# jltsiren/bwt-merge

Measured on AMD Instinct MI355X. Metric: merged Gbases/sec (input1+input2), bit-exact native BWT; value = inputs and result resident in HBM, host_to_host_value = SURVEY 8(d)'s T (page-locked host to page-locked host), higher is better.
Workload: dtype u64

## Files before the change

### bwt-merge_amd/csrc/api/context.hip.h

```cpp
#pragma once


namespace
{

thread_local std::string g_error;

int fail(int code, const char* fmt, ...)
{
  char buf[512];
  va_list ap; va_start(ap, fmt); vsnprintf(buf, sizeof(buf), fmt, ap); va_end(ap);
  g_error = buf;
  return code;
}

inline u64 div_up(u64 a, u64 b) { return (a + b - 1) / b; }

}


struct bwtm_context
{
  int device = -1;
  hipStream_t stream = nullptr;
  hipStream_t copy_stream = nullptr;
  std::recursive_mutex mu;
  bool is_default = false;
  std::atomic<long long> live_handles{0};

  bool profiling = false;
  std::string profile_only;
  bool profile_open = false;
  struct Pending { const char* name; hipEvent_t start, stop; };
  std::vector<Pending> pending;
  std::map<std::string, std::pair<double, uint64_t>> totals;
  std::vector<const char*> order;

  std::multimap<u64, void*> free_blocks;
  u64 cached_bytes = 0, held_bytes = 0, peak_bytes = 0;
  struct VBlock { u64 bytes = 0; std::vector<hipMemGenericAllocationHandle_t> chunks; hipEvent_t released = nullptr; };
  bool vmm = false;
  std::vector<hipMemGenericAllocationHandle_t> free_chunks;
  std::map<void*, VBlock> vblocks;
  u64 device_total = 0;
  u64 va_fallbacks = 0;

  void* stream_stage[4] = {nullptr, nullptr, nullptr, nullptr};
  u64 stream_stage_cap[4] = {0, 0, 0, 0};
  u64* host_scratch = nullptr;
  u64 scan1_tiles = 0, pull_scan1_tiles = 0;
};

namespace
{

struct Tuning
{
  long long search_algo = 0;
  long long frontier_unfused = 0;
  long long l1_cap = 0;
  long long emit_path = 0;
  long long round_emits = 1ll << 33;
  long long emit_budget = 0;
  long long frontier_epoch = 512;
  long long eager_cum_budget = 16ll << 30;
  long long upload_chunk = 256ll << 20;
  long long download_chunk = 128ll << 20;
  long long range_ratio = 8;
#ifdef BWTM_EXPERIMENTAL
  long long search_view = 0;
#endif
  long long frontier_stage_out = 1;
  long long frontier_parts = 0;
  long long part_capacity = 0;
  long long recs_uniform = 0;
  long long recs_window = 0;
  long long stream_samples_query = 0;
  long long stream_upload = 0;
  long long extract_batch = 1ll << 20;
  long long ingest_verify = 0;
#ifdef BWTM_DIAGNOSTICS
  long long walk_emit = 0;
  long long walk_blocks = 0;
  long long walk_kernel = 0;
  long long walk_ablate = 0;
  long long walk_variant = 0;
  long long scatter_kernel = 0;
#endif
};
Tuning g_tune;

std::mutex g_registry_mu;
std::map<int, bwtm_context*> g_default_ctx;
thread_local bwtm_context* t_bound = nullptr;
thread_local bwtm_context* t_ctx = nullptr;

#define CTX (*t_ctx)

#define HIP_TRY(expr) do { hipError_t e_ = (expr); if(e_ != hipSuccess) { \
  return fail(e_ == hipErrorOutOfMemory ? BWTM_ENOMEM : BWTM_ENODEV, "%s failed: %s (%s:%d)", #expr, hipGetErrorString(e_), __FILE__, __LINE__); } } while(0)

#define TRY(expr) do { int rc_ = (expr); if(rc_ != BWTM_OK) { return rc_; } } while(0)

void vmm_setup(bwtm_context* c);
void pool_trim(bwtm_context* c);
void stream_stage_free(bwtm_context* c)
{
  for(int k = 0; k < 4; k++) { if(c->stream_stage[k]) { (void)hipHostFree(c->stream_stage[k]); } c->stream_stage[k] = nullptr; c->stream_stage_cap[k] = 0; }
}
void apply_env_tuning();

int context_setup(bwtm_context* c, int device)
{
  int count = 0;
  hipError_t e = hipGetDeviceCount(&count);
  if(e != hipSuccess || count <= 0) { return fail(BWTM_ENODEV, "no HIP device available (%s)", hipGetErrorString(e)); }
  if(device < 0 || device >= count) { return fail(BWTM_EINVAL, "device %d out of range (%d devices)", device, count); }
  HIP_TRY(hipSetDevice(device));
  apply_env_tuning();
  c->device = device;
  HIP_TRY(hipStreamCreateWithFlags(&c->stream, hipStreamNonBlocking));
  HIP_TRY(hipStreamCreateWithFlags(&c->copy_stream, hipStreamNonBlocking));
  HIP_TRY(hipHostMalloc((void**)&c->host_scratch, 128 * sizeof(u64), hipHostMallocDefault));
  vmm_setup(c);
  {
    hipDeviceProp_t prop;
    HIP_TRY(hipGetDeviceProperties(&prop, device));
    int per_cu_scan = 0, per_cu_pull = 0;
    HIP_TRY(hipOccupancyMaxActiveBlocksPerMultiprocessor(&per_cu_scan, (const void*)k_frontier_scan1, BLOCK_THREADS, 0));
    HIP_TRY(hipOccupancyMaxActiveBlocksPerMultiprocessor(&per_cu_pull, (const void*)k_pull_scan1, BLOCK_THREADS, 0));
    c->scan1_tiles = std::min<u64>(FRONTIER_SCAN1_TILES, (u64)std::max(per_cu_scan, 0) * (u64)std::max(prop.multiProcessorCount, 0));
    c->pull_scan1_tiles = std::min<u64>(FRONTIER_SCAN1_TILES, (u64)std::max(per_cu_pull, 0) * (u64)std::max(prop.multiProcessorCount, 0));
  }
  HIP_TRY(hipFuncSetAttribute((const void*)k_part_scatter_sorted, hipFuncAttributeMaxDynamicSharedMemorySize, 96 * 1024));
  HIP_TRY(hipFuncSetAttribute((const void*)k_lf_walk_binned<true>, hipFuncAttributeMaxDynamicSharedMemorySize, 40 * 1024));
#ifdef BWTM_DIAGNOSTICS
  HIP_TRY(hipFuncSetAttribute((const void*)k_lf_walk_lds<true>, hipFuncAttributeMaxDynamicSharedMemorySize, 122 * 1024));
  HIP_TRY(hipFuncSetAttribute((const void*)k_lf_walk_lds<false>, hipFuncAttributeMaxDynamicSharedMemorySize, 82 * 1024));
#endif
  return BWTM_OK;
}

void context_teardown(bwtm_context* c)
{
  if(c->device < 0) { return; }
  (void)hipSetDevice(c->device);
  if(c->stream) { (void)hipStreamSynchronize(c->stream); }
  if(c->copy_stream) { (void)hipStreamSynchronize(c->copy_stream); }
  for(auto& p : c->pending) { (void)hipEventDestroy(p.start); (void)hipEventDestroy(p.stop); }
  c->pending.clear();
  pool_trim(c);
  stream_stage_free(c);
  if(c->host_scratch) { (void)hipHostFree(c->host_scratch); }
  if(c->stream) { (void)hipStreamDestroy(c->stream); }
  if(c->copy_stream) { (void)hipStreamDestroy(c->copy_stream); }
}

int default_context(int device, bwtm_context** out)
{
  std::lock_guard<std::mutex> lock(g_registry_mu);
  auto it = g_default_ctx.find(device);
  if(it != g_default_ctx.end()) { *out = it->second; return BWTM_OK; }
  bwtm_context* c = new bwtm_context();
  c->is_default = true;
// ... 413 lines not shown

extern "C" void bwtm_context_destroy(bwtm_context* context)
{
  if(!context || context->is_default) { return; }
  if(t_bound == context) { t_bound = nullptr; }
  if(context->live_handles.load() > 0)
  {
    fail(BWTM_EINVAL, "bwtm_context_destroy: %lld handles of the context are still alive; context not destroyed", context->live_handles.load());
    return;
  }
  context_teardown(context);
  delete context;
}

extern "C" const char* bwtm_last_error(void) { return g_error.c_str(); }

namespace
{
int tune_set(const char* key, long long value)
{
  std::string k(key);
  if(k == "search_algo") { g_tune.search_algo = value; }
  else if(k == "frontier_unfused") { g_tune.frontier_unfused = value; }
  else if(k == "l1_cap") { g_tune.l1_cap = value; }
  else if(k == "emit_path") { g_tune.emit_path = value; }
  else if(k == "round_emits") { g_tune.round_emits = (value > 0 ? value : 1); }
  else if(k == "emit_budget") { g_tune.emit_budget = (value > 0 ? value : 0); }
  else if(k == "frontier_epoch") { g_tune.frontier_epoch = (value > 0 ? value : 512); }
  else if(k == "range_ratio") { g_tune.range_ratio = (value >= 0 ? value : 8); }
#ifdef BWTM_EXPERIMENTAL
  else if(k == "search_view") { g_tune.search_view = (value >= 0 && value <= 2 ? value : 0); }
#endif
  else if(k == "frontier_stage_out") { g_tune.frontier_stage_out = (value != 0); }
  else if(k == "frontier_parts") { g_tune.frontier_parts = (value > 0 ? value : 0); }
  else if(k == "stream_samples_query") { g_tune.stream_samples_query = (value != 0); }
  else if(k == "stream_upload") { g_tune.stream_upload = (value != 0); }
  else if(k == "ingest_verify") { g_tune.ingest_verify = (value != 0); }
  else if(k == "extract_batch") { g_tune.extract_batch = (value > 0 ? value : (1ll << 20)); }
  else if(k == "part_capacity") { g_tune.part_capacity = value; }
  else if(k == "recs_uniform") { g_tune.recs_uniform = (value > 0 ? 1 : (value < 0 ? -1 : 0)); }
  else if(k == "recs_window") { g_tune.recs_window = (value == 8192 || value == 16384 || value == 32768 ? value : 0); }
  else if(k == "eager_cum_budget") { g_tune.eager_cum_budget = (value > 0 ? value : (16ll << 30)); }
  else if(k == "upload_chunk") { g_tune.upload_chunk = (value > 0 ? value : (256ll << 20)); }
  else if(k == "download_chunk") { g_tune.download_chunk = (value > 0 ? value : (128ll << 20)); }
#ifdef BWTM_DIAGNOSTICS
  else if(k == "walk_emit") { g_tune.walk_emit = value; }
  else if(k == "walk_blocks") { g_tune.walk_blocks = value; }
  else if(k == "walk_kernel") { g_tune.walk_kernel = value; }
  else if(k == "walk_ablate") { g_tune.walk_ablate = value; }
  else if(k == "walk_variant") { g_tune.walk_variant = value; }
  else if(k == "scatter_kernel") { g_tune.scatter_kernel = value; }
#endif
  else { return fail(BWTM_EINVAL, "bwtm_tune: unknown key %s", key); }
  return BWTM_OK;
}

void apply_env_tuning()
{
  static std::mutex mu;
  static bool done = false;
  std::lock_guard<std::mutex> lock(mu);
  if(done) { return; }
  done = true;
  const char* env = std::getenv("BWTM_TUNE");
  if(!env) { return; }
  std::string all(env);
// ... 124 lines not shown
```

### bwt-merge_amd/csrc/api/search.hip.h

```cpp
#pragma once

struct bwtm_ra
{
  bwtm_context* ctx = nullptr;
  bwtm_ra() : ctx(t_ctx) { if(ctx) { ctx->live_handles++; } }
  ~bwtm_ra() { if(ctx) { ctx->live_handles--; } }
  bwtm_ra(const bwtm_ra&) = delete; bwtm_ra& operator=(const bwtm_ra&) = delete;
  u64 na = 0, nb = 0, n_out = 0;
  u64 nrecs_out = 0, nchunks = 0;
  DevBuf owned_bits;
  void* bits_ptr = nullptr;
  template<class T> T* bits_as() const { return (T*)bits_ptr; }
  DevBuf chunk_base;
  bool finalized = false;
  u64 values = 0;
  bool ranged = false;
  u64 range_first = 0, range_last = 0;
  DevBuf range_rel;
  DevBuf super_boff;
  bool windowed = false;
  u64 win_word_first = 0, win_words = 0;
};

#define WHOLE_RA(ra, who) if((ra)->windowed) { return fail(BWTM_EINVAL, who ": a window of a rank array (bwtm_ra_create_range) only serves the merge over partitioned records and the output-range entry points"); }
// ... 260 lines not shown
  {
    const u64 limit = std::max<u64>(1, std::min<u64>(count / (u64)g_tune.range_ratio, 1ull << 24));
    TRY(range_phase(a, b, seq_first, count, ra, limit, levels));
    if(levels.N == 0) { return BWTM_OK; }
    TRY(range_alive(levels, node_offsets));
    count = levels.alive;
    if(count == 0) { return BWTM_OK; }
  }
  const u64 ntiles = div_up(ra->n_out + 1, 1ull << TILE_SHIFT);
  const u64 nb_max = div_up(count, FR_BLOCK);
  const u64 nseg = 5 * nb_max;
  const u64 fcap = nb_max * FR_BLOCK;

  const u64 per_seq = b->n / (b->m > 0 ? b->m : 1) + 1;
  u64 emit_budget = (u64)g_tune.emit_budget;
  if(emit_budget == 0)
  {
    emit_budget = 16ull << 30;
    size_t free_b = 0, total_b = 0;
    if(hipMemGetInfo(&free_b, &total_b) == hipSuccess) { emit_budget = std::min<u64>(std::max<u64>(emit_budget, ((u64)free_b + CTX.cached_bytes) / 2), 64ull << 30); }
    else { (void)hipGetLastError(); }
  }
  u64 emit_cap = emit_budget / sizeof(unsigned short);
  if(emit_cap > b->n + 64) { emit_cap = b->n + 64; }
  if(emit_cap > 2 * count * per_seq + (1ull << 20)) { emit_cap = 2 * count * per_seq + (1ull << 20); }
  if(emit_cap < count) { emit_cap = count; }
  u64 EPOCH = std::max<u64>(1, (u64)g_tune.frontier_epoch);
  if(g_tune.l1_cap > 0) { emit_cap = (u64)g_tune.l1_cap; }
  else { EPOCH = std::max<u64>(1, std::min<u64>(EPOCH, emit_cap / std::max<u64>(count, 1))); }
  const u64 bound_budget = 2ull << 30;
  if(EPOCH * (ntiles + 1) * sizeof(u32) > bound_budget) { EPOCH = std::max<u64>(1, bound_budget / ((ntiles + 1) * sizeof(u32))); }

  const bool wide = (a->n >= (1ull << 32) || b->n >= (1ull << 32));
  DevBuf lo[2], hi[2], seg_len[2], seg_phys[2], seg_prefix, emit16, emit_base, bound;
  for(int k = 0; k < 2; k++)
  {
    TRY(lo[k].alloc(fcap * 8)); if(wide) { TRY(hi[k].alloc(fcap * 2)); }
    TRY(seg_len[k].alloc((nseg + 1) * sizeof(u64), true)); TRY(seg_phys[k].alloc((nseg + 1) * sizeof(u64), true));
  }
  TRY(seg_prefix.alloc((nseg + 1) * sizeof(u64)));
  DevBuf first_seg; TRY(first_seg.alloc((nb_max + 1) * sizeof(u32)));
  const u32 LOOK = (count >= (1ull << 24) ? 4 : (count >= (1ull << 20) ? 8 : 32));
  struct Events
  {
    hipEvent_t ev[32]; u32 n = 0;
    ~Events() { for(u32 k = 0; k < n; k++) { (void)hipEventDestroy(ev[k]); } }
  } events;
  for(u32 k = 0; k < LOOK; k++) { HIP_TRY(hipEventCreateWithFlags(&events.ev[k], hipEventDisableTiming)); events.n = k + 1; }
  const u64 scan_tiles = div_up(nseg + 1, (u64)SCAN_TILE);
  DevBuf scan_partial; TRY(scan_partial.alloc(scan_tiles * sizeof(u64), true));
  TRY(emit16.alloc((emit_cap + 16) * sizeof(unsigned short)));
  TRY(emit_base.alloc((EPOCH + 1) * sizeof(u64), true));
  TRY(bound.alloc(EPOCH * (ntiles + 1) * sizeof(u32)));
  HIP_TRY(hipMemsetAsync(bound.p, 0xFF, EPOCH * (ntiles + 1) * sizeof(u32), CTX.stream));

  if(node_phase)
  {
    TRY(range_expand(levels, node_offsets, lo[0].as<uint2>(), hi[0].as<unsigned short>()));
    LAUNCH("frontier_init", k_frontier_init_tables, div_up(nseg + 1, BLOCK_THREADS), BLOCK_THREADS, seg_len[0].as<u64>(), seg_phys[0].as<u64>(), nb_max, count);
    levels.release(); node_offsets.release();
  }
  else
  {
    u64 init_items = (fcap > nseg + 1 ? fcap : nseg + 1);
    LAUNCH("frontier_init", k_frontier_init, div_up(init_items, BLOCK_THREADS), BLOCK_THREADS, lo[0].as<uint2>(), hi[0].as<unsigned short>(),
      seg_len[0].as<u64>(), seg_phys[0].as<u64>(), nb_max, seq_first, count, a->m);
  }
  int cur = 0;
  u64 in_epoch = 0;
  u64 alive_bound = count, epoch_used = 0;
#ifdef BWTM_EXPERIMENTAL
  bool use_view = (g_tune.search_view == 1);
  if(g_tune.search_view == 2)
  {
    const u64 steps_left = (b->m > 0 ? b->n / b->m : 0);
    size_t free_b = 0, total_b = 0;
    const u64 need = (num_view_records(a->n) + num_view_records(b->n)) * 64;
    use_view = (count >= (1ull << 22) && steps_left >= 32 && hipMemGetInfo(&free_b, &total_b) == hipSuccess && (u64)free_b + CTX.cached_bytes > need + (8ull << 30));
    (void)hipGetLastError();
  }
  if(use_view)
  {
    int rc_view = ensure_view(a);
    if(rc_view == BWTM_OK) { rc_view = ensure_view(b); }
    if(rc_view != BWTM_OK) { use_view = false; }
  }
#endif
  u64 grid = nb_max;
  u64 written[2] = {nb_max, 0};
  u64* host_ring = nullptr;
  HIP_TRY(hipHostGetDevicePointer((void**)&host_ring, CTX.host_scratch + 64, 0));
  for(u64 t = 0; t <= b->n; t++)
  {
    bool size_in_ring = false;
    if(t >= LOOK)
    {
      HIP_TRY(hipEventSynchronize(events.ev[t % LOOK]));
      alive_bound = CTX.host_scratch[64 + (u32)(t % LOOK)];
      if(alive_bound == 0) { break; }
    }
    if(scan_tiles <= CTX.scan1_tiles && g_tune.frontier_unfused == 0)
    {
      LAUNCH("frontier_scan", k_frontier_scan1, scan_tiles, BLOCK_THREADS, seg_len[cur].as<const u64>(), scan_partial.as<unsigned long long>(), (u32)((t & 0x7FFFFFFFull) + 1), nseg,
        seg_prefix.as<u64>(), first_seg.as<u32>(), emit_base.as<u64>(), in_epoch, host_ring + (t % LOOK));
      size_in_ring = true;
    }
    else if(scan_tiles <= FRONTIER_SCAN_TILES && g_tune.frontier_unfused != 1)
    {
      if(scan_tiles > 1)
      {
        LAUNCH("scan_reduce", k_scan_reduce<0>, scan_tiles, BLOCK_THREADS, seg_len[cur].as<const u64>(), scan_partial.as<u64>(), nseg + 1, (u64)0, scan_tiles);
      }
      LAUNCH("frontier_scan", k_frontier_scan, scan_tiles, BLOCK_THREADS, seg_len[cur].as<const u64>(), scan_partial.as<const u64>(), nseg,
        seg_prefix.as<u64>(), first_seg.as<u32>(), emit_base.as<u64>(), in_epoch, host_ring + (t % LOOK));
      size_in_ring = true;
    }
    else
    {
      TRY(device_scan<0>(seg_len[cur].as<u64>(), seg_prefix.as<u64>(), nseg + 1));
      LAUNCH("frontier_prep", k_frontier_prep, div_up(nseg, BLOCK_THREADS), BLOCK_THREADS, seg_prefix.as<const u64>(), nseg, first_seg.as<u32>(),
        emit_base.as<u64>(), in_epoch);
    }
    if(!size_in_ring) { TRY(fetch_u64(seg_prefix.as<u64>() + nseg, 64 + (u32)(t % LOOK))); HIP_TRY(hipEventRecord(events.ev[t % LOOK], CTX.stream)); }
    {
      const u64 need = std::max<u64>(1, div_up(alive_bound, FR_BLOCK));
      if(g_tune.frontier_parts <= 1 && need * 4 < grid * 3) { grid = need; }
      const int nxt = 1 - cur;
      if(written[nxt] > grid)
      {
        for(u64 c = 0; c < 5; c++) { HIP_TRY(hipMemsetAsync(seg_len[nxt].as<u64>() + c * nb_max + grid, 0, (written[nxt] - grid) * sizeof(u64), CTX.stream)); }
      }
      written[nxt] = grid;
    }
    FrontierView f;
    f.lo = lo[cur].as<const uint2>(); f.hi = hi[cur].as<const unsigned short>();
    f.lo_next = lo[1 - cur].as<uint2>(); f.hi_next = hi[1 - cur].as<unsigned short>();
    f.seg_prefix = seg_prefix.as<const u64>(); f.seg_phys = seg_phys[cur].as<const u64>(); f.first_seg = first_seg.as<const u32>();
    f.seg_len_next = seg_len[1 - cur].as<u64>(); f.seg_phys_next = seg_phys[1 - cur].as<u64>();
    f.nb_max = nb_max;
    f.emit16 = emit16.as<unsigned short>(); f.emit_base = emit_base.as<const u64>(); f.emit_cap = emit_cap; f.bits32 = ra->bits_as<u32>();
    f.bound_row = bound.as<u32>() + in_epoch * (ntiles + 1); f.step = in_epoch; f.block_base = 0; f.src_lo = nullptr; f.src_hi = nullptr; f.nseg_in = 0;
#ifdef BWTM_DIAGNOSTICS
    if(g_tune.walk_emit == 1 && wide) { LAUNCH_STEP("frontier_step_noemit", 1, true, false, false, grid, a->view(), b->view(), f); }
    else if(g_tune.walk_emit == 1) { LAUNCH_STEP("frontier_step_noemit", 1, false, false, false, grid, a->view(), b->view(), f); }
    else
#endif
    if(g_tune.frontier_parts > 1)
    {
      const u64 parts = (u64)g_tune.frontier_parts, per = div_up(nb_max, parts);
      for(u64 part = 0; part < parts && part * per < nb_max; part++)
      {
        f.block_base = (u32)(part * per);
        const u64 nb_part = std::min<u64>(per, nb_max - part * per);
        const char* label = (part == 0 ? "frontier_step_slice0" : "frontier_step_slices");
        if(wide) { LAUNCH_STEP(label, 0, true, false, false, nb_part, a->view(), b->view(), f); }
        else { LAUNCH_STEP(label, 0, false, false, false, nb_part, a->view(), b->view(), f); }
      }
    }
#ifdef BWTM_EXPERIMENTAL
    else if(use_view && wide) { LAUNCH_STEP("frontier_step", 0, true, true, false, grid, a->view(), b->view(), f); }
    else if(use_view) { LAUNCH_STEP("frontier_step", 0, false, true, false, grid, a->view(), b->view(), f); }
#endif
    else if(wide) { LAUNCH_STEP("frontier_step", 0, true, false, false, grid, a->view(), b->view(), f); }
    else { LAUNCH_STEP("frontier_step", 0, false, false, false, grid, a->view(), b->view(), f); }
    if(size_in_ring) { HIP_TRY(hipEventRecord(events.ev[t % LOOK], CTX.stream)); }
    cur = 1 - cur;
    in_epoch++; epoch_used += alive_bound;
    if(in_epoch == EPOCH || (g_tune.l1_cap == 0 && epoch_used + alive_bound > emit_cap))
    {
      TRY(frontier_flush(ra, emit16, emit_cap, emit_base, bound, ntiles, in_epoch));
      HIP_TRY(hipMemsetAsync(bound.p, 0xFF, EPOCH * (ntiles + 1) * sizeof(u32), CTX.stream));
      HIP_TRY(hipMemsetAsync(emit_base.p, 0, (EPOCH + 1) * sizeof(u64), CTX.stream));
      in_epoch = 0; epoch_used = 0;
    }
  }
  TRY(frontier_flush(ra, emit16, emit_cap, emit_base, bound, ntiles, in_epoch));
  return BWTM_OK;
}

}


extern "C" uint64_t bwtm_ra_buffer_bytes(const bwtm_index* a, const bwtm_index* b)
{
  if(!a || !b) { return 0; }
  return div_up(num_records(a->n + b->n), 64) * CHUNK_WORDS * sizeof(u64);
}

extern "C" int bwtm_ra_create_on(const bwtm_index* a, const bwtm_index* b, void* device_buffer, uint64_t nbytes, bwtm_ra** out)
{
  if(!a || !b || !out) { return fail(BWTM_EINVAL, "bwtm_ra_create: null argument"); }
  if(a->ctx != b->ctx) { return fail(BWTM_EINVAL, "bwtm_ra_create: the two indexes live in different contexts"); }
  ENTER(a->ctx);
  bwtm_ra* ra = new bwtm_ra();
  ra->ctx = t_ctx;
// ... 170 lines not shown
```

### bwt-merge_amd/csrc/kernels/search_frontier.hip.h

```cpp
#pragma once


constexpr int FR_BLOCK = 256;
constexpr u32 PULL_SRC_SHIFT_ = 56;
constexpr u64 PULL_PHYS_MASK_ = (1ull << PULL_SRC_SHIFT_) - 1;
constexpr int FR_SEGS = 31;

struct FrontierView
{
  const uint2* lo; const unsigned short* hi;
  uint2* lo_next; unsigned short* hi_next;
  const u64* seg_prefix;
  const u64* seg_phys;
  const u32* first_seg;
  u64* seg_len_next; u64* seg_phys_next;
  u64 nb_max;
  unsigned short* emit16;
  const u64* emit_base;
  u64 emit_cap;
  u32* bits32;
  u32* bound_row;
  u64 step;
  u32 block_base;
  const uint2* const* src_lo; const unsigned short* const* src_hi;
  u64 nseg_in;
};

__global__ void __launch_bounds__(BLOCK_THREADS) k_frontier_init(uint2* lo, unsigned short* hi, u64* seg_len, u64* seg_phys, u64 nb_max,
  u64 seq_first, u64 count, u64 m_a)
{
  u64 g = (u64)blockIdx.x * BLOCK_THREADS + threadIdx.x;
  if(g < count)
  {
    u64 i = seq_first + g;
    lo[g] = make_uint2((u32)i, (u32)m_a);
    if(hi) { hi[g] = (unsigned short)(((i >> 32) & 0xFF) | (((m_a >> 32) & 0xFF) << 8)); }
  }
  if(g < 5 * nb_max)
  {
    u64 cls = g / nb_max, b = g % nb_max;
    u64 begin = b * FR_BLOCK;
    seg_len[g] = (cls == 0 && begin < count ? (count - begin < (u64)FR_BLOCK ? count - begin : (u64)FR_BLOCK) : 0);
    seg_phys[g] = begin;
  }
  if(g == 5 * nb_max) { seg_len[g] = 0; }
}

struct RecordFetch { uint4 v[4]; };

__device__ inline RecordFetch record_issue(const uint4* recs, u64 nrecs, u64 rec)
{
  RecordFetch rf;
  const uint4* p = recs + 4 * (rec < nrecs ? rec : nrecs - 1);
  rf.v[0] = p[0]; rf.v[1] = p[1]; rf.v[2] = p[2]; rf.v[3] = p[3];
  return rf;
}

__device__ inline void record_words(const RecordFetch& rf, u32 w[16])
{
#pragma unroll
  for(int k = 0; k < 4; k++) { w[4 * k] = rf.v[k].x; w[4 * k + 1] = rf.v[k].y; w[4 * k + 2] = rf.v[k].z; w[4 * k + 3] = rf.v[k].w; }
}

__device__ inline u64 ordinary_lf(const IndexView& X, u64 pos, u32& c, bool want_symbol)
{
  const uint4* p = X.recs + 4 * (pos >> REC_SHIFT);
  const u32 j = (u32)(pos & (REC_POS - 1));
  if(want_symbol)
  {
    const uint4 ch = p[j >> 5];
    const u32 t = j & 31;
    c = ((ch.x >> t) & 1u) | (((ch.y >> t) & 1u) << 1) | (((ch.z >> t) & 1u) << 2);
  }
  if(c == 0) { return 0; }
  u32 total = 0; u32 h[4];
#pragma unroll
  for(u32 k = 0; k < 4; k++)
  {
    const uint4 ch = p[k];
    total += (u32)__builtin_popcount(plane_match(ch.x, ch.y, ch.z, c) & below_mask(j, k));
    h[k] = ch.w;
  }
  const u32 sh = FIELD_BITS * (c - 1);
  const u64 lo = (u64)h[0] | ((u64)h[1] << 32), hi = (u64)h[2] | ((u64)h[3] << 32);
  u64 v;
  if(sh < 64) { v = lo >> sh; if(sh + FIELD_BITS > 64) { v |= hi << (64 - sh); } }
  else { v = hi >> (sh - 64); }
  return X.sup[(pos >> SUPER_SHIFT) * SUP_STRIDE + c] + ((u32)v & FIELD_MASK) + total;
}

template<int EMIT, bool HI, bool VIEW = false, bool PULL = false, bool STAGE = false>
__global__ void __launch_bounds__(FR_BLOCK, (VIEW ? 6 : 8)) k_frontier_step(IndexView A, IndexView B, FrontierView f)
{
  __shared__ u32 wave_cnt[FR_BLOCK / WAVE][6];
  __shared__ uint2 s_out[STAGE ? FR_BLOCK : 1];
  __shared__ unsigned short s_out_hi[STAGE && HI ? FR_BLOCK : 1];
  __shared__ u64 s_prefix[FR_SEGS + 1], s_phys[FR_SEGS + 1];
  __shared__ const uint2* s_src_lo[PULL ? 16 : 1];
  __shared__ const unsigned short* s_src_hi[PULL ? 16 : 1];
  const u64 nseg_out = 5 * f.nb_max;
  const u64 nseg = (PULL ? f.nseg_in : nseg_out);
  const u64 N = f.seg_prefix[nseg];
  const u32 bid = blockIdx.x + f.block_base;
  const u64 g0 = (u64)bid * FR_BLOCK;
  const u32 lane = lane_id(), wave = threadIdx.x >> 6;

  if(g0 >= N)
  {
    if(threadIdx.x < 5) { f.seg_len_next[(u64)threadIdx.x * f.nb_max + bid] = 0; f.seg_phys_next[(u64)threadIdx.x * f.nb_max + bid] = g0; }
    if(bid == 0 && threadIdx.x == 5) { f.seg_len_next[nseg_out] = 0; }
    return;
  }
  const u64 first_seg = f.first_seg[bid];
  if(threadIdx.x <= FR_SEGS)
  {
    u64 sidx = first_seg + threadIdx.x; if(sidx > nseg) { sidx = nseg; }
    s_prefix[threadIdx.x] = f.seg_prefix[sidx];
    s_phys[threadIdx.x] = f.seg_phys[sidx < nseg ? sidx : nseg - 1];
  }
  if(PULL && threadIdx.x >= 64 && threadIdx.x < 80)
  {
    s_src_lo[threadIdx.x - 64] = f.src_lo[threadIdx.x - 64];
    if(HI) { s_src_hi[threadIdx.x - 64] = f.src_hi[threadIdx.x - 64]; }
  }
  __syncthreads();

  const u64 g = g0 + threadIdx.x;
  const bool active = (g < N);
  u64 i = 0, r = 0;
  if(active)
  {
    u64 phys;
    u32 k = 0;
#pragma unroll
    for(u32 step = 16; step != 0; step >>= 1) { if(s_prefix[k + step] <= g) { k += step; } }
    if(k < (u32)FR_SEGS) { phys = s_phys[k] + (g - s_prefix[k]); }
    else
    {
      u64 lo_s = first_seg + FR_SEGS, hi_s = nseg;
      while(hi_s - lo_s > 1)
      {
// ... 151 lines not shown
  {
    u32 tot = 0, bw = 0;
    for(u32 w2 = 0; w2 < FR_BLOCK / WAVE; w2++) { u32 v = wave_cnt[w2][k]; if(w2 < wave) { bw += v; } tot += v; }
    if(k < c) { class_base += tot; }
    if(k == c) { before_waves = bw; }
    tot_k[k] = tot;
  }
  if(STAGE)
  {
    if(active && c != 0)
    {
      const u32 at = class_base + before_waves + my_rank;
      s_out[at] = make_uint2((u32)ni, (u32)nr);
      if(HI) { s_out_hi[at] = (unsigned short)(((ni >> 32) & 0xFF) | (((nr >> 32) & 0xFF) << 8)); }
    }
    asm volatile("s_waitcnt lgkmcnt(0)" ::: "memory");
    __builtin_amdgcn_s_barrier();
    asm volatile("" ::: "memory");
    const u32 survivors = tot_k[1] + tot_k[2] + tot_k[3] + tot_k[4] + tot_k[5];
    const uint2 v = s_out[threadIdx.x];
    const unsigned short vh = (HI ? s_out_hi[threadIdx.x] : (unsigned short)0);
    if(threadIdx.x < survivors)
    {
      nt_store(&f.lo_next[g0 + threadIdx.x], v);
      if(HI) { nt_store(&f.hi_next[g0 + threadIdx.x], vh); }
    }
  }
  else if(active && c != 0)
  {
    u64 dst = g0 + class_base + before_waves + my_rank;
    nt_store(&f.lo_next[dst], make_uint2((u32)ni, (u32)nr));
    if(HI) { nt_store(&f.hi_next[dst], (unsigned short)(((ni >> 32) & 0xFF) | (((nr >> 32) & 0xFF) << 8))); }
  }
  if(wave == 0)
  {
    const u32 kk = threadIdx.x + 1;
    u32 tot = 0, base_k = 0;
#pragma unroll
    for(u32 k = 1; k < 6; k++) { if(k == kk) { tot = tot_k[k]; } if(k < kk) { base_k += tot_k[k]; } }
    if(kk < 6)
    {
      f.seg_len_next[(u64)(kk - 1) * f.nb_max + bid] = tot;
      f.seg_phys_next[(u64)(kk - 1) * f.nb_max + bid] = g0 + base_k;
    }
    if(bid == 0 && threadIdx.x == 5) { f.seg_len_next[nseg_out] = 0; }
  }
  if(mark_first) { atomicMin(&f.bound_row[tile_first], (u32)g); }
}

__global__ void __launch_bounds__(BLOCK_THREADS) k_frontier_prep(const u64* seg_prefix, u64 nseg, u32* first_seg, u64* emit_base, u64 step)
{
  u64 sgm = (u64)blockIdx.x * BLOCK_THREADS + threadIdx.x;
  if(sgm == 0) { emit_base[step + 1] = emit_base[step] + seg_prefix[nseg]; }
  if(sgm >= nseg) { return; }
  u64 begin = seg_prefix[sgm], end = seg_prefix[sgm + 1];
  u64 b = (begin + FR_BLOCK - 1) / FR_BLOCK;
  if(b * FR_BLOCK < end) { first_seg[b] = (u32)sgm; }
}

constexpr u64 FRONTIER_SCAN_TILES = 8192;
constexpr u64 FRONTIER_SCAN1_TILES = 1024;

__global__ void __launch_bounds__(BLOCK_THREADS) k_frontier_scan(const u64* seg_len, const u64* partial, u64 nseg, u64* seg_prefix, u32* first_seg,
  u64* emit_base, u64 step, u64* host_n)
{
  __shared__ u64 lds[BLOCK_THREADS / WAVE];
  const u64 n = nseg + 1;
  u64 c = 0;
  for(u64 k = threadIdx.x; k < blockIdx.x; k += BLOCK_THREADS) { c += partial[k]; }
  const u64 carry = block_reduce<0>(c, lds);
  const u64 base = (u64)blockIdx.x * SCAN_TILE + (u64)threadIdx.x * SCAN_ITEMS;
  u64 item[SCAN_ITEMS];
  u64 acc = 0;
#pragma unroll
  for(int k = 0; k < SCAN_ITEMS; k++) { item[k] = seg_len[base + k < n ? base + k : n - 1]; }
#pragma unroll
  for(int k = 0; k < SCAN_ITEMS; k++) { if(base + k >= n) { item[k] = 0; } acc += item[k]; }
  const u64 incl = wave_incl_sum(acc);
  const u64 wave_total = shfl_u64(incl, WAVE - 1);
  u64 excl = shfl_up_u64(incl, 1);
  if(lane_id() == 0) { excl = 0; }
  if(lane_id() == 0) { lds[threadIdx.x >> 6] = wave_total; }
  __syncthreads();
  u64 run = carry + excl;
  for(int k = 0; k < (int)(threadIdx.x >> 6); k++) { run += lds[k]; }
  for(int k = 0; k < SCAN_ITEMS; k++)
  {
    const u64 idx = base + k;
    if(idx < n)
    {
      seg_prefix[idx] = run;
      if(idx < nseg)
      {
        const u64 b = (run + FR_BLOCK - 1) / FR_BLOCK;
        if(b * FR_BLOCK < run + item[k]) { first_seg[b] = (u32)idx; }
      }
      else { emit_base[step + 1] = emit_base[step] + run; if(host_n) { *host_n = run; } }
    }
    run += item[k];
  }
}

__global__ void __launch_bounds__(BLOCK_THREADS) k_frontier_scan1(const u64* seg_len, unsigned long long* tile_total, u32 tag, u64 nseg, u64* seg_prefix, u32* first_seg,
  u64* emit_base, u64 step, u64* host_n)
{
  __shared__ u64 lds[BLOCK_THREADS / WAVE];
  const u64 n = nseg + 1;
  const u64 base = (u64)blockIdx.x * SCAN_TILE + (u64)threadIdx.x * SCAN_ITEMS;
  u64 item[SCAN_ITEMS];
  u64 acc = 0;
#pragma unroll
  for(int k = 0; k < SCAN_ITEMS; k++) { item[k] = seg_len[base + k < n ? base + k : n - 1]; }
#pragma unroll
  for(int k = 0; k < SCAN_ITEMS; k++) { if(base + k >= n) { item[k] = 0; } acc += item[k]; }
  const u64 incl = wave_incl_sum(acc);
  const u64 wave_total = shfl_u64(incl, WAVE - 1);
  u64 excl = shfl_up_u64(incl, 1);
  if(lane_id() == 0) { excl = 0; }
  if(lane_id() == 0) { lds[threadIdx.x >> 6] = wave_total; }
  __syncthreads();
  u64 before_waves = 0, tile_sum = 0;
  for(int k = 0; k < BLOCK_THREADS / WAVE; k++) { if(k < (int)(threadIdx.x >> 6)) { before_waves += lds[k]; } tile_sum += lds[k]; }
  if(threadIdx.x == 0) { __hip_atomic_store(&tile_total[blockIdx.x], ((unsigned long long)tag << 32) | (unsigned long long)tile_sum, __ATOMIC_RELAXED, __HIP_MEMORY_SCOPE_AGENT); }
  __syncthreads();
  u64 c = 0;
  for(u64 k = threadIdx.x; k < blockIdx.x; k += BLOCK_THREADS)
  {
    unsigned long long w;
    do { w = __hip_atomic_load(&tile_total[k], __ATOMIC_RELAXED, __HIP_MEMORY_SCOPE_AGENT); } while((u32)(w >> 32) != tag);
    c += (u32)w;
  }
  const u64 carry = block_reduce<0>(c, lds);
  u64 run = carry + before_waves + excl;
  for(int k = 0; k < SCAN_ITEMS; k++)
  {
    const u64 idx = base + k;
    if(idx < n)
    {
      seg_prefix[idx] = run;
      if(idx < nseg)
      {
        const u64 b = (run + FR_BLOCK - 1) / FR_BLOCK;
        if(b * FR_BLOCK < run + item[k]) { first_seg[b] = (u32)idx; }
      }
      else { emit_base[step + 1] = emit_base[step] + run; if(host_n) { *host_n = run; } }
    }
    run += item[k];
  }
}

constexpr u32 BOUND_SEG = 2048;

__global__ void __launch_bounds__(BLOCK_THREADS) k_bound_seg_min(const u32* bound, u64 ntiles, u64 nsegs, u32* segmin)
{
  __shared__ u32 lds[BLOCK_THREADS / WAVE];
  const u64 t = blockIdx.y, sg = blockIdx.x;
  const u32* row = bound + t * (ntiles + 1);
  u32 m = 0xFFFFFFFFu;
  for(u64 idx = sg * BOUND_SEG + threadIdx.x; idx < ntiles && idx < (sg + 1) * BOUND_SEG; idx += BLOCK_THREADS) { const u32 v = row[idx]; m = (v < m ? v : m); }
  m = 0xFFFFFFFFu - (u32)wave_max((u64)(0xFFFFFFFFu - m));
  if(lane_id() == 0) { lds[threadIdx.x >> 6] = m; }
  __syncthreads();
  if(threadIdx.x == 0)
  {
    for(int k = 1; k < BLOCK_THREADS / WAVE; k++) { m = (lds[k] < m ? lds[k] : m); }
    segmin[t * nsegs + sg] = m;
  }
}

__global__ void __launch_bounds__(BLOCK_THREADS) k_bound_suffix_min(u32* bound, u64 ntiles, u64 nsegs, const u32* segmin, const u64* emit_base)
{
  __shared__ u32 lds[BLOCK_THREADS];
  __shared__ u32 later[BLOCK_THREADS / WAVE];
  const u64 t = blockIdx.y, sg = blockIdx.x;
  u32* row = bound + t * (ntiles + 1);
  const u32 n_t = (u32)(emit_base[t + 1] - emit_base[t]);
  if(sg + 1 == nsegs && threadIdx.x == 0) { row[ntiles] = n_t; }
  u32 m = n_t;
  for(u64 k = sg + 1 + threadIdx.x; k < nsegs; k += BLOCK_THREADS) { const u32 v = segmin[t * nsegs + k]; m = (v < m ? v : m); }
  m = 0xFFFFFFFFu - (u32)wave_max((u64)(0xFFFFFFFFu - m));
  if(lane_id() == 0) { later[threadIdx.x >> 6] = m; }
// ... 163 lines not shown
```

### bwt-merge_amd/csrc/kernels/search_range.hip.h

```cpp
#pragma once

constexpr u32 RANGE_INLINE_WORDS = 4;
constexpr u32 RANGE_PIECE_WORDS = 2048;
constexpr u32 RANGE_EXPAND_INLINE = 48;
constexpr u32 RANGE_EXPAND_PIECE = 1024;

struct RangePiece { u64 first; u64 count; u64 aux; u64 dst; };

__device__ inline void range_set_bits(u32* bits, u64 p0, u64 p1)
{
  for(u64 w = p0 >> 5; w <= ((p1 - 1) >> 5); w++)
  {
    const u64 lo = (w << 5 > p0 ? w << 5 : p0), hi = (((w + 1) << 5) < p1 ? (w + 1) << 5 : p1);
    const u32 n = (u32)(hi - lo), sh = (u32)(lo & 31);
    const u32 mask = (n == 32 ? 0xFFFFFFFFu : ((1u << n) - 1u) << sh);
    atomicOr(bits + w, mask);
  }
}

__global__ void __launch_bounds__(BLOCK_THREADS) k_range_init(u64* sp, u64* r, u64* cnt, u64 seq_first, u64 count, u64 m_a)
{
  if(blockIdx.x == 0 && threadIdx.x == 0) { sp[0] = seq_first; r[0] = m_a; cnt[0] = count; }
}

// ... 80 lines not shown
  const u32 n = (u32)((k + RANGE_EXPAND_PIECE - 1) / RANGE_EXPAND_PIECE);
  const u32 at = atomicAdd(npieces, n);
  for(u32 q = 0; q < n; q++)
  {
    const u64 b = (u64)q * RANGE_EXPAND_PIECE;
    const u64 c = (k - b < (u64)RANGE_EXPAND_PIECE ? k - b : (u64)RANGE_EXPAND_PIECE);
    if(at + q < piece_cap) { RangePiece pc; pc.first = s + b; pc.count = c; pc.aux = rr; pc.dst = g0 + b; pieces[at + q] = pc; }
    else { for(u64 j = 0; j < c; j++) { range_store_element(lo, hi, g0 + b + j, s + b + j, rr); } }
  }
}

__global__ void __launch_bounds__(BLOCK_THREADS) k_range_expand_pieces(const RangePiece* pieces, const u32* npieces, u32 piece_cap, uint2* lo, unsigned short* hi)
{
  u32 n = *npieces; if(n > piece_cap) { n = piece_cap; }
  for(u32 q = blockIdx.x; q < n; q += gridDim.x)
  {
    const RangePiece pc = pieces[q];
    for(u64 j = threadIdx.x; j < pc.count; j += BLOCK_THREADS) { range_store_element(lo, hi, pc.dst + j, pc.first + j, pc.aux); }
  }
}

__global__ void __launch_bounds__(BLOCK_THREADS) k_frontier_init_tables(u64* seg_len, u64* seg_phys, u64 nb_max, u64 count)
{
  u64 g = (u64)blockIdx.x * BLOCK_THREADS + threadIdx.x;
  if(g < 5 * nb_max)
  {
    u64 cls = g / nb_max, b = g % nb_max;
    u64 begin = b * FR_BLOCK;
    seg_len[g] = (cls == 0 && begin < count ? (count - begin < (u64)FR_BLOCK ? count - begin : (u64)FR_BLOCK) : 0);
    seg_phys[g] = begin;
  }
  if(g == 5 * nb_max) { seg_len[g] = 0; }
}
```

Before: 90.52.

## Pack per-block frontier class counts into one word and derive segment offsets in scan

Replaces the 5-class segment length and physical-offset tables written by each frontier step with a single 64-bit word per block holding five 9-bit class counts. The scan kernels unpack these words, compute segment lengths and within-block offsets, and write the physical-offset table themselves. This removes the per-block 5x2 table writes in the step kernel and shrinks the memset of stale entries, at the cost of extra unpacking arithmetic and phys stores in the scan. It relies on per-block counts fitting in 9 bits and is enabled by default for the single-GPU path.

```diff
diff --git a/bwt-merge_amd/csrc/api/context.hip.h b/bwt-merge_amd/csrc/api/context.hip.h
--- a/bwt-merge_amd/csrc/api/context.hip.h
+++ b/bwt-merge_amd/csrc/api/context.hip.h
@@ -48,7 +48,7 @@
   void* stream_stage[4] = {nullptr, nullptr, nullptr, nullptr};
   u64 stream_stage_cap[4] = {0, 0, 0, 0};
   u64* host_scratch = nullptr;
-  u64 scan1_tiles = 0, pull_scan1_tiles = 0;
+  u64 scan1_tiles = 0, pull_scan1_tiles = 0, scan1_packed_tiles = 0;
 };
 
 namespace
@@ -71,6 +71,7 @@
   long long search_view = 0;
 #endif
   long long frontier_stage_out = 1;
+  long long frontier_pack_tables = 1;
   long long frontier_parts = 0;
   long long part_capacity = 0;
   long long recs_uniform = 0;
@@ -126,10 +127,12 @@
   {
     hipDeviceProp_t prop;
     HIP_TRY(hipGetDeviceProperties(&prop, device));
-    int per_cu_scan = 0, per_cu_pull = 0;
+    int per_cu_scan = 0, per_cu_pull = 0, per_cu_packed = 0;
     HIP_TRY(hipOccupancyMaxActiveBlocksPerMultiprocessor(&per_cu_scan, (const void*)k_frontier_scan1, BLOCK_THREADS, 0));
+    HIP_TRY(hipOccupancyMaxActiveBlocksPerMultiprocessor(&per_cu_packed, (const void*)k_frontier_scan1_packed, BLOCK_THREADS, 0));
     HIP_TRY(hipOccupancyMaxActiveBlocksPerMultiprocessor(&per_cu_pull, (const void*)k_pull_scan1, BLOCK_THREADS, 0));
     c->scan1_tiles = std::min<u64>(FRONTIER_SCAN1_TILES, (u64)std::max(per_cu_scan, 0) * (u64)std::max(prop.multiProcessorCount, 0));
+    c->scan1_packed_tiles = std::min<u64>(FRONTIER_SCAN1_TILES, (u64)std::max(per_cu_packed, 0) * (u64)std::max(prop.multiProcessorCount, 0));
     c->pull_scan1_tiles = std::min<u64>(FRONTIER_SCAN1_TILES, (u64)std::max(per_cu_pull, 0) * (u64)std::max(prop.multiProcessorCount, 0));
   }
   HIP_TRY(hipFuncSetAttribute((const void*)k_part_scatter_sorted, hipFuncAttributeMaxDynamicSharedMemorySize, 96 * 1024));
@@ -609,6 +612,7 @@
   else if(k == "search_view") { g_tune.search_view = (value >= 0 && value <= 2 ? value : 0); }
 #endif
   else if(k == "frontier_stage_out") { g_tune.frontier_stage_out = (value != 0); }
+  else if(k == "frontier_pack_tables") { g_tune.frontier_pack_tables = (value != 0); }
   else if(k == "frontier_parts") { g_tune.frontier_parts = (value > 0 ? value : 0); }
   else if(k == "stream_samples_query") { g_tune.stream_samples_query = (value != 0); }
   else if(k == "stream_upload") { g_tune.stream_upload = (value != 0); }
diff --git a/bwt-merge_amd/csrc/api/search.hip.h b/bwt-merge_amd/csrc/api/search.hip.h
--- a/bwt-merge_amd/csrc/api/search.hip.h
+++ b/bwt-merge_amd/csrc/api/search.hip.h
@@ -316,11 +316,21 @@
   if(EPOCH * (ntiles + 1) * sizeof(u32) > bound_budget) { EPOCH = std::max<u64>(1, bound_budget / ((ntiles + 1) * sizeof(u32))); }
 
   const bool wide = (a->n >= (1ull << 32) || b->n >= (1ull << 32));
-  DevBuf lo[2], hi[2], seg_len[2], seg_phys[2], seg_prefix, emit16, emit_base, bound;
+  const u64 scan_tiles = div_up(nseg + 1, (u64)SCAN_TILE);
+  bool pack = (g_tune.frontier_pack_tables != 0 && scan_tiles <= FRONTIER_SCAN_TILES && g_tune.frontier_unfused != 1 && g_tune.frontier_parts <= 1);
+#ifdef BWTM_EXPERIMENTAL
+  if(g_tune.search_view != 0) { pack = false; }
+#endif
+#ifdef BWTM_DIAGNOSTICS
+  if(g_tune.walk_emit == 1) { pack = false; }
+#endif
+  DevBuf lo[2], hi[2], seg_len[2], seg_phys[2], seg_pack[2], seg_prefix, emit16, emit_base, bound;
   for(int k = 0; k < 2; k++)
   {
     TRY(lo[k].alloc(fcap * 8)); if(wide) { TRY(hi[k].alloc(fcap * 2)); }
-    TRY(seg_len[k].alloc((nseg + 1) * sizeof(u64), true)); TRY(seg_phys[k].alloc((nseg + 1) * sizeof(u64), true));
+    if(pack) { TRY(seg_pack[k].alloc((nb_max + 1) * sizeof(u64), true)); }
+    else { TRY(seg_len[k].alloc((nseg + 1) * sizeof(u64), true)); }
+    if(!pack || k == 0) { TRY(seg_phys[k].alloc((nseg + 1) * sizeof(u64), true)); }
   }
   TRY(seg_prefix.alloc((nseg + 1) * sizeof(u64)));
   DevBuf first_seg; TRY(first_seg.alloc((nb_max + 1) * sizeof(u32)));
@@ -331,7 +341,6 @@
     ~Events() { for(u32 k = 0; k < n; k++) { (void)hipEventDestroy(ev[k]); } }
   } events;
   for(u32 k = 0; k < LOOK; k++) { HIP_TRY(hipEventCreateWithFlags(&events.ev[k], hipEventDisableTiming)); events.n = k + 1; }
-  const u64 scan_tiles = div_up(nseg + 1, (u64)SCAN_TILE);
   DevBuf scan_partial; TRY(scan_partial.alloc(scan_tiles * sizeof(u64), true));
   TRY(emit16.alloc((emit_cap + 16) * sizeof(unsigned short)));
   TRY(emit_base.alloc((EPOCH + 1) * sizeof(u64), true));
@@ -341,14 +350,23 @@
   if(node_phase)
   {
     TRY(range_expand(levels, node_offsets, lo[0].as<uint2>(), hi[0].as<unsigned short>()));
-    LAUNCH("frontier_init", k_frontier_init_tables, div_up(nseg + 1, BLOCK_THREADS), BLOCK_THREADS, seg_len[0].as<u64>(), seg_phys[0].as<u64>(), nb_max, count);
+    if(pack) { LAUNCH("frontier_init", k_frontier_init_tables_packed, div_up(nb_max + 1, BLOCK_THREADS), BLOCK_THREADS, seg_pack[0].as<u64>(), nb_max, count); }
+    else { LAUNCH("frontier_init", k_frontier_init_tables, div_up(nseg + 1, BLOCK_THREADS), BLOCK_THREADS, seg_len[0].as<u64>(), seg_phys[0].as<u64>(), nb_max, count); }
     levels.release(); node_offsets.release();
   }
   else
   {
     u64 init_items = (fcap > nseg + 1 ? fcap : nseg + 1);
-    LAUNCH("frontier_init", k_frontier_init, div_up(init_items, BLOCK_THREADS), BLOCK_THREADS, lo[0].as<uint2>(), hi[0].as<unsigned short>(),
-      seg_len[0].as<u64>(), seg_phys[0].as<u64>(), nb_max, seq_first, count, a->m);
+    if(pack)
+    {
+      LAUNCH("frontier_init", k_frontier_init_packed, div_up(init_items, BLOCK_THREADS), BLOCK_THREADS, lo[0].as<uint2>(), hi[0].as<unsigned short>(),
+        seg_pack[0].as<u64>(), nb_max, seq_first, count, a->m);
+    }
+    else
+    {
+      LAUNCH("frontier_init", k_frontier_init, div_up(init_items, BLOCK_THREADS), BLOCK_THREADS, lo[0].as<uint2>(), hi[0].as<unsigned short>(),
+        seg_len[0].as<u64>(), seg_phys[0].as<u64>(), nb_max, seq_first, count, a->m);
+    }
   }
   int cur = 0;
   u64 in_epoch = 0;
@@ -383,7 +401,23 @@
       alive_bound = CTX.host_scratch[64 + (u32)(t % LOOK)];
       if(alive_bound == 0) { break; }
     }
-    if(scan_tiles <= CTX.scan1_tiles && g_tune.frontier_unfused == 0)
+    if(pack && scan_tiles <= CTX.scan1_packed_tiles && g_tune.frontier_unfused == 0)
+    {
+      LAUNCH("frontier_scan", k_frontier_scan1_packed, scan_tiles, BLOCK_THREADS, seg_pack[cur].as<const u64>(), scan_partial.as<unsigned long long>(), (u32)((t & 0x7FFFFFFFull) + 1), nseg, nb_max,
+        seg_prefix.as<u64>(), seg_phys[0].as<u64>(), first_seg.as<u32>(), emit_base.as<u64>(), in_epoch, host_ring + (t % LOOK));
+      size_in_ring = true;
+    }
+    else if(pack)
+    {
+      if(scan_tiles > 1)
+      {
+        LAUNCH("scan_reduce", k_frontier_reduce_packed, scan_tiles, BLOCK_THREADS, seg_pack[cur].as<const u64>(), scan_partial.as<u64>(), nseg, nb_max);
+      }
+      LAUNCH("frontier_scan", k_frontier_scan_packed, scan_tiles, BLOCK_THREADS, seg_pack[cur].as<const u64>(), scan_partial.as<const u64>(), nseg, nb_max,
+        seg_prefix.as<u64>(), seg_phys[0].as<u64>(), first_seg.as<u32>(), emit_base.as<u64>(), in_epoch, host_ring + (t % LOOK));
+      size_in_ring = true;
+    }
+    else if(scan_tiles <= CTX.scan1_tiles && g_tune.frontier_unfused == 0)
     {
       LAUNCH("frontier_scan", k_frontier_scan1, scan_tiles, BLOCK_THREADS, seg_len[cur].as<const u64>(), scan_partial.as<unsigned long long>(), (u32)((t & 0x7FFFFFFFull) + 1), nseg,
         seg_prefix.as<u64>(), first_seg.as<u32>(), emit_base.as<u64>(), in_epoch, host_ring + (t % LOOK));
@@ -410,7 +444,8 @@
       const u64 need = std::max<u64>(1, div_up(alive_bound, FR_BLOCK));
       if(g_tune.frontier_parts <= 1 && need * 4 < grid * 3) { grid = need; }
       const int nxt = 1 - cur;
-      if(written[nxt] > grid)
+      if(written[nxt] > grid && pack) { HIP_TRY(hipMemsetAsync(seg_pack[nxt].as<u64>() + grid, 0, (written[nxt] - grid) * sizeof(u64), CTX.stream)); }
+      else if(written[nxt] > grid)
       {
         for(u64 c = 0; c < 5; c++) { HIP_TRY(hipMemsetAsync(seg_len[nxt].as<u64>() + c * nb_max + grid, 0, (written[nxt] - grid) * sizeof(u64), CTX.stream)); }
       }
@@ -419,8 +454,9 @@
     FrontierView f;
     f.lo = lo[cur].as<const uint2>(); f.hi = hi[cur].as<const unsigned short>();
     f.lo_next = lo[1 - cur].as<uint2>(); f.hi_next = hi[1 - cur].as<unsigned short>();
-    f.seg_prefix = seg_prefix.as<const u64>(); f.seg_phys = seg_phys[cur].as<const u64>(); f.first_seg = first_seg.as<const u32>();
+    f.seg_prefix = seg_prefix.as<const u64>(); f.seg_phys = seg_phys[pack ? 0 : cur].as<const u64>(); f.first_seg = first_seg.as<const u32>();
     f.seg_len_next = seg_len[1 - cur].as<u64>(); f.seg_phys_next = seg_phys[1 - cur].as<u64>();
+    if(pack) { f.seg_len_next = seg_pack[1 - cur].as<u64>(); f.seg_phys_next = nullptr; }
     f.nb_max = nb_max;
     f.emit16 = emit16.as<unsigned short>(); f.emit_base = emit_base.as<const u64>(); f.emit_cap = emit_cap; f.bits32 = ra->bits_as<u32>();
     f.bound_row = bound.as<u32>() + in_epoch * (ntiles + 1); f.step = in_epoch; f.block_base = 0; f.src_lo = nullptr; f.src_hi = nullptr; f.nseg_in = 0;
@@ -445,6 +481,8 @@
     else if(use_view && wide) { LAUNCH_STEP("frontier_step", 0, true, true, false, grid, a->view(), b->view(), f); }
     else if(use_view) { LAUNCH_STEP("frontier_step", 0, false, true, false, grid, a->view(), b->view(), f); }
 #endif
+    else if(pack && wide) { LAUNCH_STEP("frontier_step", FR_EMIT_PACKED, true, false, false, grid, a->view(), b->view(), f); }
+    else if(pack) { LAUNCH_STEP("frontier_step", FR_EMIT_PACKED, false, false, false, grid, a->view(), b->view(), f); }
     else if(wide) { LAUNCH_STEP("frontier_step", 0, true, false, false, grid, a->view(), b->view(), f); }
     else { LAUNCH_STEP("frontier_step", 0, false, false, false, grid, a->view(), b->view(), f); }
     if(size_in_ring) { HIP_TRY(hipEventRecord(events.ev[t % LOOK], CTX.stream)); }
diff --git a/bwt-merge_amd/csrc/kernels/search_frontier.hip.h b/bwt-merge_amd/csrc/kernels/search_frontier.hip.h
--- a/bwt-merge_amd/csrc/kernels/search_frontier.hip.h
+++ b/bwt-merge_amd/csrc/kernels/search_frontier.hip.h
@@ -46,6 +46,30 @@
   if(g == 5 * nb_max) { seg_len[g] = 0; }
 }
 
+constexpr u32 PACK_BITS = 9;
+constexpr u64 PACK_MASK = (1ull << PACK_BITS) - 1;
+
+__device__ inline u64 seg_pack_word(u32 t1, u32 t2, u32 t3, u32 t4, u32 t5)
+{
+  return (u64)t1 | ((u64)t2 << PACK_BITS) | ((u64)t3 << (2 * PACK_BITS)) | ((u64)t4 << (3 * PACK_BITS)) | ((u64)t5 << (4 * PACK_BITS));
+}
+
+__global__ void __launch_bounds__(BLOCK_THREADS) k_frontier_init_packed(uint2* lo, unsigned short* hi, u64* seg_pack, u64 nb_max, u64 seq_first, u64 count, u64 m_a)
+{
+  u64 g = (u64)blockIdx.x * BLOCK_THREADS + threadIdx.x;
+  if(g < count)
+  {
+    u64 i = seq_first + g;
+    lo[g] = make_uint2((u32)i, (u32)m_a);
+    if(hi) { hi[g] = (unsigned short)(((i >> 32) & 0xFF) | (((m_a >> 32) & 0xFF) << 8)); }
+  }
+  if(g < nb_max)
+  {
+    u64 begin = g * FR_BLOCK;
+    seg_pack[g] = (begin < count ? (count - begin < (u64)FR_BLOCK ? count - begin : (u64)FR_BLOCK) : 0);
+  }
+}
+
 struct RecordFetch { uint4 v[4]; };
 
 __device__ inline RecordFetch record_issue(const uint4* recs, u64 nrecs, u64 rec)
@@ -89,9 +113,13 @@
   return X.sup[(pos >> SUPER_SHIFT) * SUP_STRIDE + c] + ((u32)v & FIELD_MASK) + total;
 }
 
-template<int EMIT, bool HI, bool VIEW = false, bool PULL = false, bool STAGE = false>
+constexpr int FR_EMIT_PACKED = 2;
+template<int EMIT_, bool HI, bool VIEW = false, bool PULL = false, bool STAGE = false>
 __global__ void __launch_bounds__(FR_BLOCK, (VIEW ? 6 : 8)) k_frontier_step(IndexView A, IndexView B, FrontierView f)
 {
+  constexpr bool PACK = (EMIT_ == FR_EMIT_PACKED);
+  constexpr int EMIT = (PACK ? 0 : EMIT_);
+  static_assert(!(PACK && (VIEW || PULL)), "the packed table is the single-GPU search's");
   __shared__ u32 wave_cnt[FR_BLOCK / WAVE][6];
   __shared__ uint2 s_out[STAGE ? FR_BLOCK : 1];
   __shared__ unsigned short s_out_hi[STAGE && HI ? FR_BLOCK : 1];
@@ -107,6 +135,7 @@
 
   if(g0 >= N)
   {
+    if(PACK) { if(threadIdx.x == 0) { f.seg_len_next[bid] = 0; } return; }
     if(threadIdx.x < 5) { f.seg_len_next[(u64)threadIdx.x * f.nb_max + bid] = 0; f.seg_phys_next[(u64)threadIdx.x * f.nb_max + bid] = g0; }
     if(bid == 0 && threadIdx.x == 5) { f.seg_len_next[nseg_out] = 0; }
     return;
@@ -324,7 +353,11 @@
     nt_store(&f.lo_next[dst], make_uint2((u32)ni, (u32)nr));
     if(HI) { nt_store(&f.hi_next[dst], (unsigned short)(((ni >> 32) & 0xFF) | (((nr >> 32) & 0xFF) << 8))); }
   }
-  if(wave == 0)
+  if(PACK)
+  {
+    if(wave == 0) { if(threadIdx.x == 0) { f.seg_len_next[bid] = seg_pack_word(tot_k[1], tot_k[2], tot_k[3], tot_k[4], tot_k[5]); } }
+  }
+  else if(wave == 0)
   {
     const u32 kk = threadIdx.x + 1;
     u32 tot = 0, base_k = 0;
@@ -353,7 +386,63 @@
 constexpr u64 FRONTIER_SCAN_TILES = 8192;
 constexpr u64 FRONTIER_SCAN1_TILES = 1024;
 
-__global__ void __launch_bounds__(BLOCK_THREADS) k_frontier_scan(const u64* seg_len, const u64* partial, u64 nseg, u64* seg_prefix, u32* first_seg,
+__device__ __forceinline__ void scan_items_packed(const u64* seg_pack, u64 nseg, u64 nb_max, u64 base, u64 item[SCAN_ITEMS], u32 below[SCAN_ITEMS], u32& blk0)
+{
+  const u32 e0 = (u32)(base < nseg ? base : nseg - 1);
+  u32 cls[SCAN_ITEMS], blk[SCAN_ITEMS];
+  u32 k0 = e0 / (u32)nb_max, b0 = e0 - k0 * (u32)nb_max;
+  blk0 = b0;
+#pragma unroll
+  for(int k = 0; k < SCAN_ITEMS; k++)
+  {
+    cls[k] = k0; blk[k] = b0;
+    if(++b0 == (u32)nb_max) { b0 = 0; k0++; }
+  }
+  u64 w[SCAN_ITEMS];
+#pragma unroll
+  for(int k = 0; k < SCAN_ITEMS; k++) { w[k] = seg_pack[blk[k]]; }
+#pragma unroll
+  for(int k = 0; k < SCAN_ITEMS; k++)
+  {
+    u32 len = 0, bel = 0;
+#pragma unroll
+    for(u32 q = 0; q < 5; q++)
+    {
+      const u32 fq = (u32)(w[k] >> (q * PACK_BITS)) & (u32)PACK_MASK;
+      if(q < cls[k]) { bel += fq; }
+      if(q == cls[k]) { len = fq; }
+    }
+    item[k] = (base + k < nseg ? (u64)len : 0);
+    below[k] = bel;
+  }
+}
+
+__device__ __forceinline__ void store_phys_packed(u64* seg_phys, u64 nseg, u64 nb_max, u64 base, const u32 below[SCAN_ITEMS], u32 blk)
+{
+  u64 phys[SCAN_ITEMS];
+#pragma unroll
+  for(int k = 0; k < SCAN_ITEMS; k++)
+  {
+    phys[k] = (u64)blk * FR_BLOCK + below[k];
+    if(++blk == (u32)nb_max) { blk = 0; }
+  }
+  if(base + SCAN_ITEMS <= nseg)
+  {
+#pragma unroll
+    for(int k = 0; k < SCAN_ITEMS; k += 2)
+    {
+      nt_store((uint4*)(seg_phys + base + k), make_uint4((u32)phys[k], (u32)(phys[k] >> 32), (u32)phys[k + 1], (u32)(phys[k + 1] >> 32)));
+    }
+  }
+  else
+  {
+#pragma unroll
+    for(int k = 0; k < SCAN_ITEMS; k++) { if(base + k < nseg) { nt_store(&seg_phys[base + k], phys[k]); } }
+  }
+}
+
+template<bool PACK>
+__device__ __forceinline__ void frontier_scan_body(const u64* seg_len, const u64* partial, u64 nseg, u64 nb_max, u64* seg_prefix, u64* seg_phys, u32* first_seg,
   u64* emit_base, u64 step, u64* host_n)
 {
   __shared__ u64 lds[BLOCK_THREADS / WAVE];
@@ -363,11 +452,22 @@
   const u64 carry = block_reduce<0>(c, lds);
   const u64 base = (u64)blockIdx.x * SCAN_TILE + (u64)threadIdx.x * SCAN_ITEMS;
   u64 item[SCAN_ITEMS];
+  u32 below[SCAN_ITEMS], blk = 0;
   u64 acc = 0;
-#pragma unroll
-  for(int k = 0; k < SCAN_ITEMS; k++) { item[k] = seg_len[base + k < n ? base + k : n - 1]; }
-#pragma unroll
-  for(int k = 0; k < SCAN_ITEMS; k++) { if(base + k >= n) { item[k] = 0; } acc += item[k]; }
+  if(PACK)
+  {
+    scan_items_packed(seg_len, nseg, nb_max, base, item, below, blk);
+    store_phys_packed(seg_phys, nseg, nb_max, base, below, blk);
+#pragma unroll
+    for(int k = 0; k < SCAN_ITEMS; k++) { acc += item[k]; }
+  }
+  else
+  {
+#pragma unroll
+    for(int k = 0; k < SCAN_ITEMS; k++) { item[k] = seg_len[base + k < n ? base + k : n - 1]; }
+#pragma unroll
+    for(int k = 0; k < SCAN_ITEMS; k++) { if(base + k >= n) { item[k] = 0; } acc += item[k]; }
+  }
   const u64 incl = wave_incl_sum(acc);
   const u64 wave_total = shfl_u64(incl, WAVE - 1);
   u64 excl = shfl_up_u64(incl, 1);
@@ -393,18 +493,56 @@
   }
 }
 
-__global__ void __launch_bounds__(BLOCK_THREADS) k_frontier_scan1(const u64* seg_len, unsigned long long* tile_total, u32 tag, u64 nseg, u64* seg_prefix, u32* first_seg,
+__global__ void __launch_bounds__(BLOCK_THREADS) k_frontier_scan(const u64* seg_len, const u64* partial, u64 nseg, u64* seg_prefix, u32* first_seg,
   u64* emit_base, u64 step, u64* host_n)
+{
+  frontier_scan_body<false>(seg_len, partial, nseg, 0, seg_prefix, nullptr, first_seg, emit_base, step, host_n);
+}
+
+__global__ void __launch_bounds__(BLOCK_THREADS) k_frontier_scan_packed(const u64* seg_pack, const u64* partial, u64 nseg, u64 nb_max, u64* seg_prefix, u64* seg_phys,
+  u32* first_seg, u64* emit_base, u64 step, u64* host_n)
+{
+  frontier_scan_body<true>(seg_pack, partial, nseg, nb_max, seg_prefix, seg_phys, first_seg, emit_base, step, host_n);
+}
+
+__global__ void __launch_bounds__(BLOCK_THREADS) k_frontier_reduce_packed(const u64* seg_pack, u64* partial, u64 nseg, u64 nb_max)
+{
+  __shared__ u64 lds[BLOCK_THREADS / WAVE];
+  const u64 base = (u64)blockIdx.x * SCAN_TILE + (u64)threadIdx.x * SCAN_ITEMS;
+  u64 item[SCAN_ITEMS];
+  u32 below[SCAN_ITEMS], blk = 0;
+  scan_items_packed(seg_pack, nseg, nb_max, base, item, below, blk);
+  u64 acc = 0;
+#pragma unroll
+  for(int k = 0; k < SCAN_ITEMS; k++) { acc += item[k]; }
+  const u64 total = block_reduce<0>(acc, lds);
+  if(threadIdx.x == 0) { partial[blockIdx.x] = total; }
+}
+
+template<bool PACK>
+__device__ __forceinline__ void frontier_scan1_body(const u64* seg_len, unsigned long long* tile_total, u32 tag, u64 nseg, u64 nb_max, u64* seg_prefix, u64* seg_phys,
+  u32* first_seg, u64* emit_base, u64 step, u64* host_n)
 {
   __shared__ u64 lds[BLOCK_THREADS / WAVE];
   const u64 n = nseg + 1;
   const u64 base = (u64)blockIdx.x * SCAN_TILE + (u64)threadIdx.x * SCAN_ITEMS;
   u64 item[SCAN_ITEMS];
+  u32 below[SCAN_ITEMS], blk = 0;
   u64 acc = 0;
-#pragma unroll
-  for(int k = 0; k < SCAN_ITEMS; k++) { item[k] = seg_len[base + k < n ? base + k : n - 1]; }
-#pragma unroll
-  for(int k = 0; k < SCAN_ITEMS; k++) { if(base + k >= n) { item[k] = 0; } acc += item[k]; }
+  if(PACK)
+  {
+    scan_items_packed(seg_len, nseg, nb_max, base, item, below, blk);
+    store_phys_packed(seg_phys, nseg, nb_max, base, below, blk);
+#pragma unroll
+    for(int k = 0; k < SCAN_ITEMS; k++) { acc += item[k]; }
+  }
+  else
+  {
+#pragma unroll
+    for(int k = 0; k < SCAN_ITEMS; k++) { item[k] = seg_len[base + k < n ? base + k : n - 1]; }
+#pragma unroll
+    for(int k = 0; k < SCAN_ITEMS; k++) { if(base + k >= n) { item[k] = 0; } acc += item[k]; }
+  }
   const u64 incl = wave_incl_sum(acc);
   const u64 wave_total = shfl_u64(incl, WAVE - 1);
   u64 excl = shfl_up_u64(incl, 1);
@@ -439,6 +577,18 @@
     }
     run += item[k];
   }
+}
+
+__global__ void __launch_bounds__(BLOCK_THREADS) k_frontier_scan1(const u64* seg_len, unsigned long long* tile_total, u32 tag, u64 nseg, u64* seg_prefix, u32* first_seg,
+  u64* emit_base, u64 step, u64* host_n)
+{
+  frontier_scan1_body<false>(seg_len, tile_total, tag, nseg, 0, seg_prefix, nullptr, first_seg, emit_base, step, host_n);
+}
+
+__global__ void __launch_bounds__(BLOCK_THREADS) k_frontier_scan1_packed(const u64* seg_pack, unsigned long long* tile_total, u32 tag, u64 nseg, u64 nb_max, u64* seg_prefix,
+  u64* seg_phys, u32* first_seg, u64* emit_base, u64 step, u64* host_n)
+{
+  frontier_scan1_body<true>(seg_pack, tile_total, tag, nseg, nb_max, seg_prefix, seg_phys, first_seg, emit_base, step, host_n);
 }
 
 constexpr u32 BOUND_SEG = 2048;
diff --git a/bwt-merge_amd/csrc/kernels/search_range.hip.h b/bwt-merge_amd/csrc/kernels/search_range.hip.h
--- a/bwt-merge_amd/csrc/kernels/search_range.hip.h
+++ b/bwt-merge_amd/csrc/kernels/search_range.hip.h
@@ -136,3 +136,13 @@
   }
   if(g == 5 * nb_max) { seg_len[g] = 0; }
 }
+
+__global__ void __launch_bounds__(BLOCK_THREADS) k_frontier_init_tables_packed(u64* seg_pack, u64 nb_max, u64 count)
+{
+  u64 g = (u64)blockIdx.x * BLOCK_THREADS + threadIdx.x;
+  if(g < nb_max)
+  {
+    u64 begin = g * FR_BLOCK;
+    seg_pack[g] = (begin < count ? (count - begin < (u64)FR_BLOCK ? count - begin : (u64)FR_BLOCK) : 0);
+  }
+}
```

After: 92.09 (median of 6 runs). 1.02x the previous value.
